# josephg/text-crdt-rust

Measured on AMD Instinct MI355X. Metric: CRDT ops remapped+merged/sec (whole node), higher is better.
Workload: dtype u32

## Files before the change

include/crdt_gpu.h:

```cpp
#ifndef CRDT_GPU_H
#define CRDT_GPU_H
#include <stddef.h>
#include <stdint.h>

#ifdef __cplusplus
extern "C" {
#endif

#define CRDT_OK 0
#define CRDT_ERR_POS_OOB -1
#define CRDT_ERR_SEQ -2
#define CRDT_ERR_UNKNOWN_AGENT -3
#define CRDT_ERR_UNKNOWN_ID -4
#define CRDT_ERR_NONTERMINATING -5
#define CRDT_ERR_CAPACITY -6
#define CRDT_ERR_EMPTY_TXN -7
#define CRDT_ERR_FRONTIER -8
#define CRDT_ERR_BAD_INPUT -9
#define CRDT_ERR_INTERNAL -10

#define CRDT_E_ARG -100
#define CRDT_E_DEVICE -101
#define CRDT_E_NOMEM -102
#define CRDT_E_WIRE -103
// ... 160 lines not shown

int crdt_doc_len(crdt_engine* e, uint64_t n, const uint32_t* doc, uint32_t* len);
int crdt_doc_status(crdt_engine* e, int32_t* status );
int crdt_digest(crdt_engine* e, uint64_t* per_doc );
int crdt_canon_counts(crdt_engine* e, uint32_t* per_doc );

int crdt_export_sizes(crdt_engine* e, uint32_t doc, uint64_t* sizes);
int crdt_export(crdt_engine* e, uint32_t doc, uint32_t* raw4, uint32_t* leaf_sizes, uint32_t* canon4,
                uint32_t* cwo4, uint32_t* del3, uint32_t* dd3, uint32_t* txn5, uint32_t* parents,
                uint32_t* frontier);

int crdt_fit(crdt_engine* e);
int crdt_fit_note(crdt_engine* e, int apply);
int crdt_reseed_random_async(crdt_engine* e, uint64_t seed, uint64_t id_base);
int crdt_digest_dev_async(crdt_engine* e, uint64_t* dev_out);
int crdt_set_share_streams(crdt_engine* e, int on);
int crdt_set_device_intern(crdt_engine* e, int on);
enum { CRDT_QUERY_LDS = 0, CRDT_QUERY_PER_THREAD = 1, CRDT_QUERY_MERGE = 2 };
int crdt_set_query_kernel(crdt_engine* e, int mode);
int crdt_set_fused_publish(crdt_engine* e, int on);
int crdt_fused_publish_stats(crdt_engine* e, uint64_t* launches, uint8_t* per_doc);
enum { CRDT_BALANCE_OFF = 0, CRDT_BALANCE_ON = 1, CRDT_BALANCE_AUTO = 2, CRDT_BALANCE_ROTATE = 3 };
int crdt_set_replay_balance(crdt_engine* e, int mode);
#define CRDT_BALANCE_BOARD_WORDS (16384u * 16u)
int crdt_debug_balance_board(crdt_engine* e, uint32_t* board, uint32_t* stamp, int* policy);
int crdt_debug_vpos(crdt_engine* e, uint32_t doc, uint32_t* vpos);
int crdt_debug_publish_plan(crdt_engine* e, uint8_t* plan, uint32_t* words);
uint64_t crdt_mem_bytes(const crdt_engine* e);
int crdt_device_bytes(uint64_t* current, uint64_t* peak, int reset_peak);
int crdt_test_fail_alloc_after(long long k);
typedef struct { uint32_t pos, agent, seq; } crdt_probe;
typedef struct { uint32_t agent, seq, pos, deleted; } crdt_probe_answer;
int crdt_apply_local_probed(crdt_engine* e, uint64_t n_docs, const uint32_t* docs, const uint64_t* txn_off,
                            const crdt_local_txn* txns, const crdt_local_op* ops, const crdt_probe* probes,
                            crdt_probe_answer* answers, int32_t* doc_status);
int crdt_debug_state(crdt_engine* e, uint32_t doc, uint32_t* out23);
int crdt_last_timings(crdt_engine* e, double* replay_ms, double* publish_ms);
void* crdt_stream(crdt_engine* e);
const char* crdt_last_error(void);
const char* crdt_build_id(void);

#ifdef __cplusplus
}
#endif
#endif
```

text-crdt-rust_amd/crdt_amd/__init__.py:

```python
from __future__ import annotations

import ctypes as C
import os
import subprocess
from typing import Iterable, Sequence

import numpy as np

PKG_DIR = os.path.dirname(os.path.abspath(__file__))
PKG_ROOT = os.path.dirname(PKG_DIR)
REPO = os.path.dirname(PKG_ROOT)
LIB_PATH = os.path.join(PKG_ROOT, "build", "libcrdt_gpu.so")
CSRC = os.path.join(PKG_ROOT, "csrc")
INCLUDE = os.path.join(REPO, "include")

OK = 0
STATUS_NAMES = {0: "OK", -1: "POS_OOB", -2: "SEQ", -3: "UNKNOWN_AGENT", -4: "UNKNOWN_ID", -5: "NONTERMINATING",
                -6: "CAPACITY", -7: "EMPTY_TXN", -8: "FRONTIER", -9: "BAD_INPUT", -10: "INTERNAL"}
ROOT_AGENT = 0xFFFF
ROOT_ORDER = 0xFFFFFFFF


class CrdtError(RuntimeError):
    pass
# ... 25 lines not shown
    if not force and os.path.exists(out) and os.path.exists(stamp):
        with open(stamp) as f:
            if f.read().strip() == hsh:
                return out
    os.makedirs(os.path.dirname(out), exist_ok=True)
    cmd = _build_cmd(out, list(defines) + [f'CRDT_SRC_HASH="{hsh}"'])
    r = subprocess.run(cmd, capture_output=not verbose, text=True)
    if r.returncode != 0:
        raise CrdtError("hipcc failed:\n" + (r.stderr or "")[-4000:])
    if not defines:
        check_codegen(out + ".tmp")
    os.replace(out + ".tmp", out)
    with open(stamp, "w") as f:
        f.write(hsh + "\n")
    return out


def build_id(path: str = None) -> str:
    L = lib() if path is None else C.CDLL(path)
    L.crdt_build_id.restype = C.c_char_p
    return L.crdt_build_id().decode()


SCRATCH_STORES_MAX = {"k_replay": 4}
CODEGEN_LIMITS = {
    "k_replay": {"vgpr_count": 64, "vgpr_spill_count": 16, "private_segment_fixed_size": 32},
    "k_replay_hr": {"vgpr_count": 128, "vgpr_spill_count": 0, "private_segment_fixed_size": 0},
    "k_publish": {"vgpr_count": 64, "vgpr_spill_count": 0, "private_segment_fixed_size": 0},
}
LLVM_BIN = "/opt/rocm/lib/llvm/bin"


def kernel_resources(lib_path: str) -> dict:
    import re
    import tempfile
    import shutil
    with tempfile.TemporaryDirectory() as td:
        cp = os.path.join(td, "lib.so")
        shutil.copyfile(lib_path, cp)
        r = subprocess.run([os.path.join(LLVM_BIN, "llvm-objdump"), "--offloading", cp], capture_output=True, text=True)
        cos = [f for f in os.listdir(td) if "amdgcn-amd-amdhsa--gfx950" in f]
        if r.returncode != 0 or not cos:
            raise CrdtError("no gfx950 code object in " + lib_path + ": " + (r.stderr or "")[-500:])
        notes = subprocess.run([os.path.join(LLVM_BIN, "llvm-readelf"), "--notes", os.path.join(td, cos[0])],
                               capture_output=True, text=True, check=True).stdout
    out, cur = {}, {}
    for line in notes.splitlines():
        m = re.match(r"\s*-?\s*\.(\w+):\s+(\S+)\s*$", line)
        if not m:
# ... 95 lines not shown
    L.crdt_apply_remote_wire.argtypes = [vp, u64, P(u32), P(C.c_char_p), P(u64), P(i32)]
    L.crdt_stage_remote_wire.argtypes = [vp, u64, P(u32), P(C.c_char_p), P(u64)]
    L.crdt_stage_remote_replicated.argtypes = [vp, C.c_char_p, u64, u32, P(C.c_char_p)]
    L.crdt_stage_random.argtypes = [vp, u64, P(u32), C.c_char_p, u32, u64]
    L.crdt_stage_local_shared.argtypes = [vp, u64, P(u32), P(u32), u32, P(u64), vp, vp]
    L.crdt_debug_state.argtypes = [vp, u32, P(u32)]
    L.crdt_fit.argtypes = [vp]
    for f, at in (("crdt_fit_note", [vp, C.c_int]), ("crdt_test_fail_alloc_after", [C.c_longlong]),
                  ("crdt_reseed_random_async", [vp, u64, u64]), ("crdt_digest_dev_async", [vp, vp])):
        if hasattr(L, f):
            getattr(L, f).argtypes = at
    L.crdt_set_share_streams.argtypes = [vp, C.c_int]
    for f in ("crdt_set_device_intern", "crdt_set_query_kernel", "crdt_set_fused_publish"):
        if hasattr(L, f):
            getattr(L, f).argtypes = [vp, C.c_int]
    if hasattr(L, "crdt_fused_publish_stats"):
        L.crdt_fused_publish_stats.argtypes = [vp, P(u64), P(C.c_uint8)]
        L.crdt_debug_vpos.argtypes = [vp, u32, P(u32)]
    if hasattr(L, "crdt_debug_publish_plan"):
        L.crdt_debug_publish_plan.argtypes = [vp, P(C.c_uint8), P(u32)]
    if hasattr(L, "crdt_set_replay_balance"):
        L.crdt_set_replay_balance.argtypes = [vp, C.c_int]
        L.crdt_debug_balance_board.argtypes = [vp, P(u32), P(u32), P(C.c_int)]
    L.crdt_apply_local_probed.argtypes = [vp, u64, P(u32), P(u64), vp, vp, vp, vp, P(i32)]
    L.crdt_mem_bytes.argtypes = [vp]
    L.crdt_mem_bytes.restype = u64
    if hasattr(L, "crdt_device_bytes"):
        L.crdt_device_bytes.argtypes = [P(u64), P(u64), C.c_int]
    L.crdt_reset_async.argtypes = [vp]
    L.crdt_run.argtypes = [vp, P(i32)]
    L.crdt_run_async.argtypes = [vp]
    L.crdt_publish_async.argtypes = [vp]
    L.crdt_sync.argtypes = [vp]
    L.crdt_pos_to_loc.argtypes = [vp, u64, P(u32), P(u32), P(C.c_uint16), P(u32)]
    L.crdt_loc_to_pos.argtypes = [vp, u64, P(u32), P(C.c_uint16), P(u32), P(u32), P(C.c_uint8)]
    L.crdt_pos_to_loc_dev_async.argtypes = [vp, u64, vp, vp, vp, vp]
    L.crdt_loc_to_pos_dev_async.argtypes = [vp, u64, vp, vp, vp, vp, vp]
    L.crdt_doc_len.argtypes = [vp, u64, P(u32), P(u32)]
    L.crdt_doc_status.argtypes = [vp, P(i32)]
    L.crdt_digest.argtypes = [vp, P(u64)]
    if hasattr(L, "crdt_canon_counts"):
        L.crdt_canon_counts.argtypes = [vp, P(u32)]
    L.crdt_export_sizes.argtypes = [vp, u32, P(u64)]
    L.crdt_export.argtypes = [vp, u32] + [P(u32)] * 9
    L.crdt_last_timings.argtypes = [vp, P(C.c_double), P(C.c_double)]
    L.crdt_stream.argtypes = [vp]
# ... 68 lines not shown

EXPORTED_SYMBOLS = [
    "crdt_engine_create", "crdt_engine_destroy", "crdt_docs_alloc", "crdt_num_docs", "crdt_agent_intern", "crdt_agent_intern_dev",
    "crdt_apply_local", "crdt_apply_remote_wire", "crdt_stage_local", "crdt_stage_remote_wire",
    "crdt_stage_remote_replicated", "crdt_reset_async", "crdt_run", "crdt_run_async", "crdt_publish_async",
    "crdt_sync", "crdt_pos_to_loc", "crdt_loc_to_pos", "crdt_pos_to_loc_dev_async", "crdt_loc_to_pos_dev_async",
    "crdt_doc_len", "crdt_doc_status", "crdt_digest", "crdt_export_sizes", "crdt_export", "crdt_last_timings",
    "crdt_stream", "crdt_last_error", "crdt_build_id", "crdt_stage_random", "crdt_debug_state",
    "crdt_stage_local_shared", "crdt_set_content", "crdt_materialize_async", "crdt_text", "crdt_text_digest",
    "crdt_last_materialize_ms", "crdt_set_content_copies", "crdt_canon_counts", "crdt_fit", "crdt_mem_bytes", "crdt_apply_local_probed", "crdt_set_share_streams", "crdt_set_device_intern", "crdt_set_query_kernel", "crdt_device_bytes",
    "crdt_fit_note", "crdt_reseed_random_async", "crdt_digest_dev_async", "crdt_test_fail_alloc_after",
    "crdt_doc_version", "crdt_diff_async", "crdt_diff_between_async", "crdt_diff_counts", "crdt_diff_read", "crdt_last_diff_ms",
    "crdt_checkout_async", "crdt_checkout_lens", "crdt_checkout_read", "crdt_checkout_digest", "crdt_pos_to_loc_at",
    "crdt_loc_to_pos_at", "crdt_pos_to_loc_at_dev_async", "crdt_loc_to_pos_at_dev_async", "crdt_last_checkout_ms",
    "crdt_blame_async", "crdt_blame_counts", "crdt_blame_read", "crdt_last_blame_ms",
    "crdt_encode_async", "crdt_encode_lens", "crdt_encode_read", "crdt_pos_to_units", "crdt_units_to_pos",
    "crdt_pos_to_units_dev_async", "crdt_units_to_pos_dev_async", "crdt_last_encode_ms",
    "crdt_lines_async", "crdt_line_counts", "crdt_lines_read", "crdt_pos_to_linecol", "crdt_linecol_to_pos",
    "crdt_pos_to_linecol_dev_async", "crdt_linecol_to_pos_dev_async", "crdt_last_lines_ms",
    "crdt_find_async", "crdt_find_counts", "crdt_find_read", "crdt_find_seek", "crdt_find_seek_dev_async", "crdt_last_find_ms",
    "crdt_edits_async", "crdt_edits_counts", "crdt_edits_read", "crdt_last_edits_ms",
    "crdt_rebase_async", "crdt_rebase_counts", "crdt_rebase_read", "crdt_rebase", "crdt_rebase_dev_async", "crdt_last_rebase_ms",
    "crdt_set_fused_publish", "crdt_fused_publish_stats", "crdt_debug_vpos", "crdt_debug_publish_plan",
    "crdt_set_replay_balance", "crdt_debug_balance_board",
    "crdt_trace_load", "crdt_trace_parse", "crdt_trace_sizes", "crdt_trace_copy", "crdt_trace_free",
]


def _p(a, t=C.c_uint32):
    return a.ctypes.data_as(C.POINTER(t))


def _check(rc: int, what: str):
    if rc != 0:
        err = lib().crdt_last_error()
        raise CrdtError(f"{what} failed rc={rc} {err.decode() if err else ''}")


class Engine:

    def __init__(self, n_docs: int, leaf_cap: int = 32, device: int = 0):
        L = lib()
        self.L = L
        self.h = C.c_void_p()
        cfg = L.Cfg(leaf_cap, device)
        _check(L.crdt_engine_create(C.byref(cfg), C.byref(self.h)), "crdt_engine_create")
        _check(L.crdt_docs_alloc(self.h, n_docs), "crdt_docs_alloc")
# ... 150 lines not shown

    QUERY_KERNELS = {"lds": 0, "per_thread": 1, "merge": 2}

    def query_kernel(self, mode: str):
        _check(self.L.crdt_set_query_kernel(self.h, self.QUERY_KERNELS[mode]), "query_kernel")

    def device_intern(self, on: bool = True):
        _check(self.L.crdt_set_device_intern(self.h, int(on)), "device_intern")

    def fused_publish(self, on: bool = True):
        _check(self.L.crdt_set_fused_publish(self.h, int(on)), "fused_publish")

    def fused_publish_stats(self):
        n = C.c_uint64()
        per = np.zeros(self.n_docs, np.uint8)
        _check(self.L.crdt_fused_publish_stats(self.h, C.byref(n), _p(per, C.c_uint8)), "fused_publish_stats")
        return n.value, per.astype(bool)

    BALANCE_MODES = {"off": 0, "on": 1, "auto": 2, "rotate": 3}

    def replay_balance(self, mode="auto"):
        _check(self.L.crdt_set_replay_balance(self.h, int(self.BALANCE_MODES.get(mode, mode))), "replay_balance")

    def balance_board(self):
        board = np.zeros((16384, 16), np.uint32)
        stamp, policy = C.c_uint32(), C.c_int()
        _check(self.L.crdt_debug_balance_board(self.h, _p(board), C.byref(stamp), C.byref(policy)), "debug_balance_board")
        return board, stamp.value, policy.value

    def debug_vpos(self, doc: int) -> np.ndarray:
        out = np.zeros(max(int(self.canon_counts()[doc]), 1), np.uint32)
        _check(self.L.crdt_debug_vpos(self.h, doc, _p(out)), "debug_vpos")
        return out[: int(self.canon_counts()[doc])]

    def publish_plan(self):
        plan = np.zeros(self.n_docs, np.uint8)
        words = np.zeros(self.n_docs, np.uint32)
        _check(self.L.crdt_debug_publish_plan(self.h, _p(plan, C.c_uint8), _p(words)), "debug_publish_plan")
        return plan, words

    def mem_bytes(self) -> int:
        return int(self.L.crdt_mem_bytes(self.h))

    @staticmethod
    def device_bytes(reset_peak: bool = False):
        cur, peak = C.c_uint64(), C.c_uint64()
# ... 610 lines not shown
```

text-crdt-rust_amd/csrc/engine.hip:

```cpp
#include <hip/hip_runtime.h>

#include <algorithm>
#include <cstdio>
#include <cstring>
#include <map>
#include <mutex>
#include <string>
#include <unordered_map>
#include <vector>

#include "crdt_gpu.h"
#include "host_plan.h"
#include "kernels.h"
#include "encode.h"
#include "lines.h"
#include "find.h"
#include "edits.h"
#include "rebase.h"

using namespace crdt;

namespace {

thread_local std::string g_last_error;
// ... 285 lines not shown
  u64* cbase = nullptr;
  u64* clen = nullptr;
  u32* text = nullptr;
  u64 text_cap = 0;
  u64 ord_total = 0;
  Span* canon = nullptr;
  u32* vpos = nullptr;
  u32* sorted = nullptr;
  u32* corder = nullptr;
  u32* pub = nullptr;
  u64 canon_alloc = 0, pub_alloc = 0;
  bool pub_sized = false;
  bool pub_fitted = false;
  std::vector<u32> pub_small, pub_big;
  u32* pub_list = nullptr;
  u32 pubx_words = 0;
  u32* stamp = nullptr;
  u64 fused_launches = 0;
  u32 state_id = 1;
  bool fused_publish = !(getenv("CRDT_NO_FUSED_PUBLISH") && getenv("CRDT_NO_FUSED_PUBLISH")[0] == '1');
  u32* bal_board = nullptr;
  int replay_balance = getenv("CRDT_REPLAY_BALANCE") && getenv("CRDT_REPLAY_BALANCE")[0] >= '0' && getenv("CRDT_REPLAY_BALANCE")[0] <= '3'
                           ? getenv("CRDT_REPLAY_BALANCE")[0] - '0' : CRDT_BALANCE_AUTO;
  u32 n_cus = 0;
  u32 bal_last_stamp = 0, bal_last_mode = BAL_OFF;
  u32 balance_mode(const RootClass& c, const LaunchShape& sh) const {
    if (replay_balance == CRDT_BALANCE_OFF) return BAL_OFF;
    if (replay_balance == CRDT_BALANCE_ROTATE) return BAL_ROTATE;
    if (replay_balance == CRDT_BALANCE_ON) return BAL_BOARD;
    const u64 by_regs = 4ull * (c.shape == SHAPE_GEN ? CRDT_REPLAY_WAVES_GEN : CRDT_REPLAY_WAVES);
    const u64 by_lds = (163840ull / std::max<size_t>(sh.lds, 1)) * sh.wpb;
    return c.n <= std::min(by_regs, by_lds) * n_cus ? BAL_ROTATE : BAL_OFF;
  }
  void state_changed() {
    if (++state_id == STAMP_BIG) {
      state_id = 1;
      pub_sized = pub_fitted = false;
    }
  }
  u32* tlen = nullptr;
  u64* tdigest = nullptr;
  bool materialized = false;
  void* qbuf = nullptr;
  u64 qbuf_bytes = 0;
  ResultJob<DiffRes, 2> diff;
  std::vector<u32> diff_docs_h, diff_since_h, diff_to_h;
// ... 640 lines not shown
    return 0;
  }

  int launch_replay() {
    if (!n_docs) return 0;
    Pools pv = pools_view(pools);
    state_changed();
    bal_last_stamp = state_id % 255u + 1u;
    bal_last_mode = BAL_OFF;
    const bool fuse = fused_publish && pub_sized && pub_fitted;
    for (const RootClass& c : classes) {
      LaunchShape sh = launch_shape(c.rcap, c.hr);
      u32 blocks = (u32)((c.n + sh.wpb - 1) / sh.wpb);
      const u32* list = c.off == INVALID ? nullptr : doc_list + c.off;
      if (c.hr) {
        if (L == 32) hipLaunchKernelGGL(k_replay_hr<32>, dim3(blocks), dim3(64 * sh.wpb), sh.lds, stream, pv, (u32)c.n, sh.wpb, sh.rcap, list);
        else hipLaunchKernelGGL(k_replay_hr<4>, dim3(blocks), dim3(64 * sh.wpb), sh.lds, stream, pv, (u32)c.n, sh.wpb, sh.rcap, list);
      } else {
        const u32 bal = balance_mode(c, sh);
        bal_last_mode = std::max(bal_last_mode, bal);
        ReplayArgs ra{pv, (u32)c.n, sh.wpb, sh.rcap, list, pub_view(), pubx_words, fuse ? state_id : 0u,
                      bal_board, bal_last_stamp, bal};
        if (L == 32) {
          if (c.shape == SHAPE_REMOTE) hipLaunchKernelGGL((k_replay<32, SHAPE_REMOTE>), dim3(blocks), dim3(64 * sh.wpb), sh.lds, stream, ra);
          else if (c.shape == SHAPE_GEN) hipLaunchKernelGGL((k_replay<32, SHAPE_GEN>), dim3(blocks), dim3(64 * sh.wpb), sh.lds, stream, ra);
          else if (c.shape == SHAPE_LOCAL) hipLaunchKernelGGL((k_replay<32, SHAPE_LOCAL>), dim3(blocks), dim3(64 * sh.wpb), sh.lds, stream, ra);
          else hipLaunchKernelGGL((k_replay<32, SHAPE_ALL>), dim3(blocks), dim3(64 * sh.wpb), sh.lds, stream, ra);
        } else {
          if (c.shape == SHAPE_REMOTE) hipLaunchKernelGGL((k_replay<4, SHAPE_REMOTE>), dim3(blocks), dim3(64 * sh.wpb), sh.lds, stream, ra);
          else if (c.shape == SHAPE_GEN) hipLaunchKernelGGL((k_replay<4, SHAPE_GEN>), dim3(blocks), dim3(64 * sh.wpb), sh.lds, stream, ra);
          else if (c.shape == SHAPE_LOCAL) hipLaunchKernelGGL((k_replay<4, SHAPE_LOCAL>), dim3(blocks), dim3(64 * sh.wpb), sh.lds, stream, ra);
          else hipLaunchKernelGGL((k_replay<4, SHAPE_ALL>), dim3(blocks), dim3(64 * sh.wpb), sh.lds, stream, ra);
        }
      }
      HIPCHK(hipGetLastError());
    }
    for (const RootClass& c : classes) if (fuse && !c.hr) { fused_launches++; break; }
    if (!pub_fitted) pub_sized = false;
    published = false;
    materialized = false;
    return 0;
  }

  int pull_states() {
    HIPCHK(hipMemcpyAsync(st_h.data(), st, n_docs * sizeof(DocState), hipMemcpyDeviceToHost, stream));
    HIPCHK(hipStreamSynchronize(stream));
    return 0;
  }

  int run(int32_t* status_out) {
    int r = set_device();
    if (r) return r;
// ... 891 lines not shown
  *out = nullptr;
  int n = 0;
  if (hipGetDeviceCount(&n) != hipSuccess || n <= cfg->device || cfg->device < 0) return CRDT_E_DEVICE;
  hipDeviceProp_t prop;
  if (hipGetDeviceProperties(&prop, cfg->device) != hipSuccess) return CRDT_E_DEVICE;
  if (std::strncmp(prop.gcnArchName, "gfx950", 6) != 0) return CRDT_E_DEVICE;
  crdt_engine* e = new crdt_engine();
  e->L = cfg->leaf_cap;
  e->device = cfg->device;
  bool ok = hipSetDevice(e->device) == hipSuccess && hipStreamCreateWithFlags(&e->stream, hipStreamNonBlocking) == hipSuccess;
  for (auto& x : e->ev) ok = ok && hipEventCreate(&x) == hipSuccess;
  e->each_job([&](auto& j) { ok = ok && j.create(e->device, e->stream) == 0; });
  e->n_cus = (u32)prop.multiProcessorCount;
  ok = ok && hipMalloc((void**)&e->bal_board, (size_t)BAL_ROWS * BAL_SLOTS * 4) == hipSuccess &&
       hipMemsetAsync(e->bal_board, 0, (size_t)BAL_ROWS * BAL_SLOTS * 4, e->stream) == hipSuccess;
  if (!ok) {
    crdt_engine_destroy(e);
    return CRDT_E_DEVICE;
  }
  (void)hipFuncSetAttribute((const void*)k_replay<32, SHAPE_ALL>, hipFuncAttributeMaxDynamicSharedMemorySize, 163840);
  (void)hipFuncSetAttribute((const void*)k_replay<4, SHAPE_ALL>, hipFuncAttributeMaxDynamicSharedMemorySize, 163840);
  (void)hipFuncSetAttribute((const void*)k_replay<32, SHAPE_REMOTE>, hipFuncAttributeMaxDynamicSharedMemorySize, 163840);
  (void)hipFuncSetAttribute((const void*)k_replay<4, SHAPE_REMOTE>, hipFuncAttributeMaxDynamicSharedMemorySize, 163840);
  (void)hipFuncSetAttribute((const void*)k_replay<32, SHAPE_GEN>, hipFuncAttributeMaxDynamicSharedMemorySize, 163840);
  (void)hipFuncSetAttribute((const void*)k_replay<32, SHAPE_LOCAL>, hipFuncAttributeMaxDynamicSharedMemorySize, 163840);
  (void)hipFuncSetAttribute((const void*)k_replay<4, SHAPE_GEN>, hipFuncAttributeMaxDynamicSharedMemorySize, 163840);
  (void)hipFuncSetAttribute((const void*)k_replay<4, SHAPE_LOCAL>, hipFuncAttributeMaxDynamicSharedMemorySize, 163840);
  (void)hipFuncSetAttribute((const void*)k_replay_hr<32>, hipFuncAttributeMaxDynamicSharedMemorySize, 163840);
  (void)hipFuncSetAttribute((const void*)k_replay_hr<4>, hipFuncAttributeMaxDynamicSharedMemorySize, 163840);
  (void)hipFuncSetAttribute((const void*)k_pos_to_loc_blk<32>, hipFuncAttributeMaxDynamicSharedMemorySize, QBLK_LDS);
  (void)hipFuncSetAttribute((const void*)k_pos_to_loc_blk<4>, hipFuncAttributeMaxDynamicSharedMemorySize, QBLK_LDS);
  (void)hipFuncSetAttribute((const void*)k_loc_to_pos_blk<32>, hipFuncAttributeMaxDynamicSharedMemorySize, QBLK_W * 8u);
  (void)hipFuncSetAttribute((const void*)k_loc_to_pos_blk<4>, hipFuncAttributeMaxDynamicSharedMemorySize, QBLK_W * 8u);
  (void)hipFuncSetAttribute((const void*)k_pub_index, hipFuncAttributeMaxDynamicSharedMemorySize,
                            (int)pubx_lds_bytes(PUBX_MAX_WORDS));
  (void)hipFuncSetAttribute((const void*)k_diff_mark, hipFuncAttributeMaxDynamicSharedMemorySize, (int)(DIFF_MARK_WORDS * 4u));
  *out = e;
  return 0;
}

void crdt_engine_destroy(crdt_engine* e) {
  if (!e) return;
  (void)hipSetDevice(e->device);
  if (e->stream) (void)hipStreamSynchronize(e->stream);
  e->release();
  if (e->bal_board) (void)hipFree(e->bal_board);
// ... 403 lines not shown
  if (!e) return CRDT_E_ARG;
  e->share_streams = on != 0;
  return 0;
}

int crdt_set_query_kernel(crdt_engine* e, int mode) {
  if (!e || mode < CRDT_QUERY_LDS || mode > CRDT_QUERY_MERGE) return CRDT_E_ARG;
  e->query_kernel = mode;
  return 0;
}

int crdt_set_fused_publish(crdt_engine* e, int on) {
  if (!e) return CRDT_E_ARG;
  e->fused_publish = on != 0;
  return 0;
}

int crdt_set_replay_balance(crdt_engine* e, int mode) {
  if (!e || mode < CRDT_BALANCE_OFF || mode > CRDT_BALANCE_ROTATE) return CRDT_E_ARG;
  e->replay_balance = mode;
  return 0;
}

int crdt_debug_balance_board(crdt_engine* e, uint32_t* board, uint32_t* stamp, int* policy) {
  if (poisoned(e)) return CRDT_E_NOMEM;
  if (!valid(e)) return CRDT_E_ARG;
  if (stamp) *stamp = e->bal_last_stamp;
  if (policy) *policy = (int)e->bal_last_mode;
  if (board) {
    HIPCHK(hipMemcpyAsync(board, e->bal_board, (size_t)BAL_ROWS * BAL_SLOTS * 4, hipMemcpyDeviceToHost, e->stream));
    HIPCHK(hipStreamSynchronize(e->stream));
  }
  return 0;
}

int crdt_fused_publish_stats(crdt_engine* e, uint64_t* launches, uint8_t* per_doc) {
  if (poisoned(e)) return CRDT_E_NOMEM;
  if (!valid(e)) return CRDT_E_ARG;
  if (launches) *launches = e->fused_launches;
  if (per_doc && e->n_docs) {
    std::vector<u32> st(e->n_docs);
    HIPCHK(hipMemcpyAsync(st.data(), e->stamp, e->n_docs * 4, hipMemcpyDeviceToHost, e->stream));
    HIPCHK(hipStreamSynchronize(e->stream));
    for (u64 d = 0; d < e->n_docs; d++) per_doc[d] = st[d] == e->state_id;
  }
  return 0;
// ... 1167 lines not shown
```

text-crdt-rust_amd/csrc/kernels.h:

```cpp
#pragma once
#include "replay_core.h"
#include "wave_gpu.h"

namespace crdt {

struct PubOut {
  Span* canon;
  u32* vpos;
  u32* sorted;
  u32* corder;
  u32* pub;
  u32* canon_n;
  u32* len;
  u64* digest;
  u32* stamp;
};
constexpr u32 STAMP_BIG = 0xFFFFFFFFu;

#ifdef PUB_PLAIN_LOADS
__device__ __forceinline__ u32 ld_l2(const u32* p) { return *p; }
#else
__device__ __forceinline__ u32 ld_l2(const u32* p) { return __hip_atomic_load(p, __ATOMIC_RELAXED, __HIP_MEMORY_SCOPE_AGENT); }
#endif
__device__ __forceinline__ u32 span_of_order(const PubOut& O, const DocSeg& seg, u32 cn, u32 order) {
// ... 34 lines not shown
  u32 d;
  if (!wave_doc(wpb, nullptr, n, d)) return;
  Replayer<WaveGPU<L>, L> r(P, d, wave_with_root<L>(rcap));
  r.init_empty();
  AgentRec* ag = r.agents();
  for (u32 a = lane_id(); a < r.g(S_N_AGENTS); a += 64) ag[a].run_cnt = 0;
  r.finish();
}

struct ReplayArgs {
  Pools P;
  u32 n, wpb, rcap;
  const u32* list;
  PubOut O;
  u32 xw, pub_id;
  u32* bal_board;
  u32 bal_stamp;
  u32 bal_mode;
};
template <int L>
__device__ __forceinline__ void publish_tail(const DocState* stp);
__device__ __forceinline__ void balance_done();

template <int L, bool HR, u32 SH = SHAPE_ALL, bool FUSE = false>
__device__ __forceinline__ void replay_doc(Pools P, u32 n, u32 wpb, u32 rcap, const u32* list) {
  u32 d;
  if (!wave_doc(wpb, list, n, d)) return;
#ifdef CRDT_PROF
  const u32 life_t0 = (u32)__builtin_amdgcn_s_memrealtime();
#endif
  Replayer<WaveGPU<L, HR>, L> r(P, d, wave_with_root<L, HR>(rcap));
  WaveGPU<L, HR>& w = r.w;
  if (r.status() == ST_NEED_CAPACITY) r.p(S_STATUS, (u32)ST_OK);
  if (r.status() != ST_OK || r.g(S_REC_POS) >= r.rec_n()) {
    w.st((u32*)&P.st[d].status, (u32)r.status());
    if constexpr (!HR) balance_done();
    return;
  }
  r.begin();
  r.template run<SH>();
  r.finish();
#ifdef CRDT_PROF
  __builtin_amdgcn_fence(__ATOMIC_RELEASE, "workgroup");
  const u32 life_t1 = (u32)__builtin_amdgcn_s_memrealtime();
#endif
  if constexpr (!HR) balance_done();
  if constexpr (FUSE) publish_tail<L>(r.stp());
#ifdef CRDT_PROF
  if (r.prof_mode == 4u) {
    __builtin_amdgcn_fence(__ATOMIC_RELEASE, "workgroup");
    const u32 tail = (u32)__builtin_amdgcn_s_memrealtime() - life_t1;
    w.st(&P.st[d].prof0, life_t0);
    w.st(&P.st[d].prof1, life_t1);
    w.st(&P.st[d].prof2, (u32)__builtin_amdgcn_s_getreg(4 | (31 << 11)));
    w.st(&P.st[d].prof3, ((u32)__builtin_amdgcn_s_getreg(20 | (31 << 11)) & 15u) | (tail << 4));
  }
#endif
}
#ifndef CRDT_REPLAY_WAVES
#define CRDT_REPLAY_WAVES 8
#endif
#ifndef CRDT_REPLAY_WAVES_GEN
#define CRDT_REPLAY_WAVES_GEN CRDT_REPLAY_WAVES
#endif
template <int L, u32 SH>
__global__ __launch_bounds__(256) __attribute__((amdgpu_waves_per_eu(SH == SHAPE_GEN ? CRDT_REPLAY_WAVES_GEN : CRDT_REPLAY_WAVES))) void k_replay(ReplayArgs A) {
  replay_doc<L, false, SH, true>(A.P, A.n, A.wpb, A.rcap, A.list);
}
template <int L>
__global__ __launch_bounds__(256) __attribute__((amdgpu_waves_per_eu(4))) void k_replay_hr(Pools P, u32 n, u32 wpb, u32 rcap, const u32* list) {
  replay_doc<L, true>(P, n, wpb, rcap, list);
}

__global__ void k_reseed_gen(Pools P, u32 n, u64 seed, u64 id_base) {
  u32 d = blockIdx.x * blockDim.x + threadIdx.x;
  if (d >= n) return;
  DocSeg sg = P.seg[d];
  if (sg.rec_n != 1u) return;
  Rec* r = const_cast<Rec*>(P.recs + sg.rec_base);
  if (rec_kind(*r) != REC_GEN) return;
  r->w3 = (u32)mix64(seed ^ (id_base + d));
}

__global__ void k_reset_recpos(DocState* st, u32 n, u32 n_agents_dummy) {
  u32 d = blockIdx.x * blockDim.x + threadIdx.x;
  if (d < n) st[d].rec_pos = 0;
}

__global__ void k_set_n_agents(DocState* st, const u32* na, u32 n) {
  u32 d = blockIdx.x * blockDim.x + threadIdx.x;
// ... 2283 lines not shown
```

text-crdt-rust_amd/csrc/replay_core.h:

```cpp
#pragma once
#include "crdt_types.h"

namespace crdt {

struct Cursor {
  u32 leaf, idx, off;
};
constexpr u32 END_LEAF = 0xFFFFFFFEu;

enum : u32 {
  P_LV = 0, P_DL = 2, P_DV = 4, P_SOL = 6, P_LOF = 8, P_CWO = 10, P_ARUN = 12, P_DELS = 14,
  P_DD = 16, P_TXNS = 18, P_PAR = 20, P_FR = 22, P_AGENTS = 24, P_GROUPS = 26, P_RECS = 28, P_STP = 30,
  P_DDB = 32,
  P_PROBE = P_DDB + 2,
  K_LEAF = P_PROBE + 2, K_MAP, K_CWO, K_TXN, K_DEL, K_DD, K_PAR, K_RECN,
  K_FR,
  P_OAG,
  K_AGMAP = P_OAG + 2,
  P_LAG,
  S_BASE = 64,
  S_STATUS = 64, S_REC_POS, S_N_LEAVES, S_N_BLOCKS, S_NG, S_NEXT_ORDER, S_LEN, S_N_CWO, S_N_DEL,
  S_N_DD, S_N_TXN, S_N_PAR, S_N_FR, S_N_AGENTS, S_N_ITEMS, S_CAP_NEED, S_N_ENTRIES, S_GEN_DONE, S_N_DDB,
  S_PROF0, S_PROF1, S_PROF2, S_PROF3,
  F_FAST,
  F_PRE, PRE_ITEM, PRE_C = PRE_ITEM + 4,
  F_GEN = PRE_C + 3,
  T_RB_BASE,
  F_BASE,
  FR_S0 = 104,
  C_LEAF = 128, C_N, C_VIS, C_NOW, C_BLK, C_I, C_VSTART, C_DIRTY, C_VS_OK ,
  C_SUCC, C_SUCC_ORD,
  T_CWO_KEY, T_CWO_AGENT, T_CWO_SEQ, T_CWO_LEN,
  T_DEL_KEY, T_DEL_ORDER, T_DEL_LEN,
  T_TX_ORDER, T_TX_LEN, T_TX_SHADOW,
  T_FR0,
  T_AG_ID, T_AG_BASE, T_AG_CNT, T_AG_CAP,
  T_AGL_KEY, T_AGL_ORDER, T_AGL_LEN,
  T_OA_ID, T_OA_BASE, T_OA_CNT,
  T_AGP_KEY, T_AGP_ORDER, T_AGP_LEN,
  T_OA_KEY, T_OA_ORDER, T_OA_LEN,
  N_SLOTS
};
static_assert(P_LAG + 1 < 64, "read-only slots live in the first context register");
static_assert(S_PROF3 - S_BASE + 1 == sizeof(DocState) / 4, "DocState slot mirror");
static_assert(F_BASE < FR_S0, "DocState and the flags live in the second context register, below the frontier heads");
constexpr u32 FR_LANES = 128u - FR_S0;
static_assert(N_SLOTS <= 192, "three context registers");

template <class W, int L>
struct Replayer {
  W w;
  u32 cpt = 0;
  CRDT_HD u32 per_txn(u32 remote) const { return cpt ? 1u : (remote ? 3u : 2u); }
  CRDT_HD Rec op_at(u32 b, u32 remote) const {
    Rec r = w.rec_get(cpt ? b : b + 1u);
    if (!cpt) return r;
    Rec h, o, pr;
    if (remote) expand_rc(r, h, o, pr);
    else expand_lc(r, h, o);
    return o;
  }
#ifdef CRDT_PROF
  u32 prof_cat = 0;
  u32 prof_mode = 0;
  u32 prof_gen = 0;
  u32 prof_cur = 0, prof_sw = 0;
  u64 prof_t2 = 0;
  u32 prof_split = 0;
  u32 pt_scan = 0, pt_del = 0, pt_ins = 0;
#endif
#ifdef CRDT_EMU_STATS
  u32 st_prev_leaf = INVALID;
// ... 75 lines not shown
    p(K_AGMAP, (sg.flags & DOC_TRACK_AGENT) ? 1u : 0u);
    w.x_load_state(P.st + d, S_BASE);
    p(C_LEAF, INVALID);
    p(C_N, 0);
    p(C_VIS, 0);
    p(C_NOW, 0);
    p(C_BLK, 0);
    p(C_I, 0);
    p(C_VSTART, VS_BAD);
    p(C_DIRTY, 0);
    p(C_SUCC, INVALID);
    p(C_SUCC_ORD, 0);
    p(T_CWO_KEY, 0); p(T_CWO_AGENT, 0); p(T_CWO_SEQ, 0); p(T_CWO_LEN, 0);
    p(T_DEL_KEY, INVALID); p(T_DEL_ORDER, 0); p(T_DEL_LEN, 0);
    p(T_TX_ORDER, 0); p(T_TX_LEN, 0); p(T_TX_SHADOW, 0);
    p(T_FR0, ROOT_ORDER);
    p(T_AG_ID, INVALID); p(T_AG_BASE, 0); p(T_AG_CNT, 0); p(T_AG_CAP, 0);
    p(T_AGL_KEY, 0); p(T_AGL_ORDER, 0); p(T_AGL_LEN, 0); p(T_AGP_LEN, 0);
    p(T_OA_ID, INVALID); p(T_OA_BASE, 0); p(T_OA_CNT, 0);
    p(T_RB_BASE, 0x80000000u);
    p(F_FAST, 0);
    p(F_PRE, 0);
    p(F_GEN, 0);
  }

  CRDT_HD Span* leafp(u32 leaf) const { return w.template at<L>(lv(), leaf); }
  CRDT_HD u32* dleaf(u32 blk) const { return w.template at<GROUP>(dl(), blk); }
  CRDT_HD u32* dvis(u32 blk) const { return w.template at<GROUP>(dv(), blk); }

  CRDT_HD void init_empty() {
    p(S_STATUS, (u32)ST_OK);
    p(S_REC_POS, 0);
    p(S_N_LEAVES, 1);
    p(S_N_BLOCKS, 1);
    p(S_NG, 1);
    p(S_NEXT_ORDER, 0);
    p(S_LEN, 0);
    p(S_N_CWO, 0); p(S_N_DEL, 0); p(S_N_DD, 0); p(S_N_TXN, 0); p(S_N_PAR, 0);
    p(S_N_FR, 1);
    p(S_N_ITEMS, 0);
    p(S_CAP_NEED, 0);
    p(S_N_ENTRIES, 0);
    p(S_GEN_DONE, 0);
    p(S_N_DDB, 0);
    w.zero_leaf(leafp(0), L);
    lag_stale(0u);
// ... 52 lines not shown
    if (n <= FR_LANES + 1u) w.fr_lanes_store(fr(), n);
  }
  CRDT_HD void flush_agent() {
    u32 a = g(T_AG_ID), cnt = g(T_AG_CNT);
    if (a != INVALID && cnt) {
      u32 ln = g(T_AGL_LEN);
      w.st(&w.at(arun(), g(T_AG_BASE) + cnt - 1)->len, ln);
      w.st_agent_tail(w.at(agents(), a), g(T_AGL_KEY), g(T_AGL_ORDER), ln);
    }
  }
  CRDT_HD void finish() {
    commit();
    flush_tails();
    w.root_store(groups(), g(S_NG));
    w.x_store_state(stp(), S_BASE);
  }

  template <class X> static CRDT_HD auto tick_of(X& x, u32 remaining, int) -> decltype(x.balance_tick(remaining)) {
    x.balance_tick(remaining);
  }
  template <class X> static CRDT_HD void tick_of(X&, u32, long) {}
  CRDT_HD void balance_tick(u32 remaining) { tick_of(w, remaining, 0); }

  CRDT_HD void rec_window(u32 base) {
    u32 d = base - g(T_RB_BASE);
    u32 nn = rec_n() - base;
    balance_tick(nn);
    u32 ahead = nn > 64u ? nn - 64u : 0u;
    if (d <= 64u) w.rec_slide(d, recs() + base + 64u, ahead < 64u ? ahead : 64u);
    else w.rec_load2(recs() + base, nn < 64u ? nn : 64u, ahead < 64u ? ahead : 64u);
    p(T_RB_BASE, base);
  }
  CRDT_HD Rec rec(u32 pos) {
    u32 base = g(T_RB_BASE);
    u32 d = pos - base;
    if (d > 61u) rec_window(d <= 64u ? pos : (d < 125u ? base + 64u : pos));
    return w.rec_get(pos - g(T_RB_BASE));
  }
  CRDT_HD Rec rec_at(u32 pos) const {
    u32 d = pos - g(T_RB_BASE);
    return d < 64u ? w.rec_get(d) : w.ld_rec(w.at(recs(), pos));
  }

  CRDT_HD void slot_of(u32 leaf, u32& blk, u32& i) const {
    if (leaf == g(C_LEAF)) { blk = g(C_BLK); i = g(C_I); return; }
    u32 v = w.ld(w.template at<2>(sol(), leaf));
    blk = v >> 6;
    i = v & 63u;
  }
  CRDT_HD u32 pos_key(u32 leaf) const {
    u32 blk, i;
    slot_of(leaf, blk, i);
    return (w.root_find_blk(g(S_NG), blk) << 6) | i;
  }
// ... 1115 lines not shown
    if (g(T_FR0) != first - 1u) return 0;
    if (g(S_N_TXN) == 0u) return 0;
    return g(T_TX_ORDER) + g(T_TX_LEN) == first;
  }
  CRDT_HD void fast_txn_commit(u32 first, u32 len) {
    if (!g(F_FAST)) {
      p(F_BASE, first);
      p(F_FAST, 1u);
    }
    p(S_NEXT_ORDER, first + len);
    inc(T_AGL_LEN, len);
  }
  CRDT_HD u32 next_item_after(u32 idx, u32& order) {
    if (idx + 1u < g(C_N)) { order = w.cget_order(idx + 1u); return 1u; }
    u32 fo;
    u32 has = cached_succ(fo) != INVALID;
    order = fo;
    return has;
  }
  CRDT_HD u32 typing_run(u32 b0, u32 nv, u32 remote, u32 agent, u32 ow1, const Rec& o, u32& total) {
    u32 nt = 1u;
    total = remote ? (o.w0 & 0x0FFFFFFFu) : o.w3;
    if (!nv) return nt;
    nt = w.typing_scan(b0, nv, remote, cpt, agent, ow1, o.w3, total);
    u32 per = per_txn(remote), rn = rec_n();
    u32 pos0 = g(T_RB_BASE) + b0;
    u32 end = g(T_RB_BASE) + nv;
    while (true) {
      if (pos0 + (nt + 1u) * per <= end) break;
      if (end >= rn) break;
      u32 last = pos0 + (nt - 1u) * per;
      u32 n = rn - last < 64u ? rn - last : 64u;
      u32 t2, l0;
      u32 n2 = w.typing_scan_at(w.at(recs(), last), n, remote, cpt, agent, ow1, o.w3, t2, l0);
      end = last + n;
      if (n2 <= 1u) break;
      total += t2 - l0;
      nt += n2 - 1u;
    }
    return nt;
  }
  CRDT_HD u32 fast_typing(u32 b0, u32 nv, u32 remote, u32 idx, u32 orr, u32 agent, const Rec& o, u32 first) {
    Span e = w.cget(idx);
    if (e.len <= 0) return 0;
    if (e.order + (u32)e.len != first) return 0;
    if (e.orr != orr) return 0;
    u32 total;
// ... 929 lines not shown
```

text-crdt-rust_amd/csrc/wave_gpu.h:

```cpp
#pragma once
#include "crdt_types.h"

namespace crdt {

__device__ __forceinline__ u32 lane_id() { return __lane_id(); }
__device__ __forceinline__ u32 lane_here() {
  u32 l;
  asm volatile("v_mbcnt_lo_u32_b32 %0, -1, 0\n\tv_mbcnt_hi_u32_b32 %0, -1, %0" : "=v"(l));
  return l;
}
__device__ __forceinline__ u32 uni(u32 x) { return __builtin_amdgcn_readfirstlane(x); }
__device__ __forceinline__ u32 rdlane(u32 x, u32 l) { return __builtin_amdgcn_readlane(x, l); }
__device__ int crdt_writelane_i32(int v, int l, int old) __asm("llvm.amdgcn.writelane.i32");
__device__ __forceinline__ u32 wrlane(u32 old, u32 v, u32 l) { return (u32)crdt_writelane_i32((int)v, (int)l, (int)old); }
__device__ __forceinline__ u64 ballot(bool p) { return __builtin_amdgcn_ballot_w64(p); }
__device__ __forceinline__ u32 shfl(u32 v, u32 src) { return __builtin_amdgcn_ds_bpermute((int)(src << 2), (int)v); }

__device__ __forceinline__ u32 wave_umax(u32 v) {
  v = max(v, (u32)__builtin_amdgcn_update_dpp(0u, v, 0x111, 0xf, 0xf, false));
  v = max(v, (u32)__builtin_amdgcn_update_dpp(0u, v, 0x112, 0xf, 0xf, false));
  v = max(v, (u32)__builtin_amdgcn_update_dpp(0u, v, 0x114, 0xf, 0xf, false));
  v = max(v, (u32)__builtin_amdgcn_update_dpp(0u, v, 0x118, 0xf, 0xf, false));
  v = max(v, (u32)__builtin_amdgcn_update_dpp(0u, v, 0x142, 0xa, 0xf, false));
  v = max(v, (u32)__builtin_amdgcn_update_dpp(0u, v, 0x143, 0xc, 0xf, false));
// ... 659 lines not shown
    u32 l = lane();
    u32 d = (rx ^ ((REC_LC << 28) | agent)) | ry | rz | (rw ^ len);
    u64 stop = ballot(d != 0u || l >= nv) & (~1ull << b0);
    u32 f = stop ? (u32)__builtin_ctzll(stop) : 64u;
    return f - b0;
  }
  __device__ __forceinline__ u32 typing_scan(u32 b0, u32 nv, u32 remote, u32 compact, u32 agent, u32 ow1, u32 ow3,
                                             u32& total) const {
    return typing_scan_r(rx, ry, rz, rw, b0, nv, remote, compact, agent, ow1, ow3, total);
  }
  __device__ __forceinline__ u32 typing_scan_at(const Rec* p, u32 nv, u32 remote, u32 compact, u32 agent, u32 ow1,
                                                u32 ow3, u32& total, u32& len0) const {
    uint4 v = rec_lane_load(p, nv);
    len0 = (compact & remote) ? (rdlane(v.x, 0) >> 16) & 0x7FFu : rdlane(v.w, 0);
    return typing_scan_r(v.x, v.y, v.z, v.w, 0u, nv, remote, compact, agent, ow1, ow3, total);
  }
  __device__ __forceinline__ u32 delete_scan(u32 b0, u32 nv, u32 remote, u32 compact, u32 agent, u32 delta) const {
    return delete_scan_r(rx, ry, rz, rw, b0, nv, remote, compact, agent, delta);
  }
  __device__ __forceinline__ u32 delete_scan_at(const Rec* p, u32 nv, u32 remote, u32 compact, u32 agent, u32 delta) const {
    uint4 v = rec_lane_load(p, nv);
    return delete_scan_r(v.x, v.y, v.z, v.w, 0u, nv, remote, compact, agent, delta);
  }
  __device__ __forceinline__ u32 frontier_advance(u32* f, u32 nfr, u32 f0, const u32* pp, u32 np, u32 p0, u32 first,
                                                  u32 last, u32 cap, u32& nf0) const {
    u32 l = lane();
    bool in = l < nfr;
    u32 fv = f[in ? l : 0u];
    fv = l == 0u ? f0 : fv;
    if (ballot(in && fv == first)) return 0u;
    u32 pv = np > 1u ? pp[l < np ? l : 0u] : 0u;
    pv = l == 0u ? p0 : pv;
    bool hit = false;
    for (u32 j = 0; j < np; j++) hit |= fv == rdlane(pv, j);
    u64 keep = ballot(in && !hit);
    u32 m = (u32)__popcll(keep);
    if (m + 1u > cap) return INVALID;
    nf0 = m ? rdlane(fv, (u32)__builtin_ctzll(keep)) : last;
    u32 at = (u32)__popcll(keep & ((1ull << l) - 1ull));
    if (((keep >> l) & 1ull) && at >= 1u) f[at] = fv;
    if (m) f[m] = last;
    return m + 1u;
  }
  static constexpr u32 FR_L0 = FR_S0 - 64u;
  __device__ __forceinline__ void fr_lanes_load(const u32* f, u32 n) {
    u32 l = lane();
// ... 462 lines not shown
```

Baseline: 33.48 billion.

## Precompute typing-run mask per record window in remote replay kernel

Adds a remote-only replay kernel variant that, each time the record window is loaded or slid, compares every lane's record with its neighbour via DPP and ballots a bitmask of records that continue a typing run. The mask is stored in context-register slots. For compact remote ops the typing scan then finds the run length with a count-trailing-zeros on that mask instead of running the full per-op typing scan. This trades some extra work per window refill for cheaper scans per op, and adds a new kernel instance with its own register budget. It is on by default and can be turned off with an environment variable.

Result: faster. 34.27 billion (median of 6 runs) (+2.4%).

```diff
diff --git a/include/crdt_gpu.h b/include/crdt_gpu.h
--- a/include/crdt_gpu.h
+++ b/include/crdt_gpu.h
@@ -206,6 +206,7 @@
 int crdt_fused_publish_stats(crdt_engine* e, uint64_t* launches, uint8_t* per_doc);
 enum { CRDT_BALANCE_OFF = 0, CRDT_BALANCE_ON = 1, CRDT_BALANCE_AUTO = 2, CRDT_BALANCE_ROTATE = 3 };
 int crdt_set_replay_balance(crdt_engine* e, int mode);
+int crdt_set_window_decode(crdt_engine* e, int on);
 #define CRDT_BALANCE_BOARD_WORDS (16384u * 16u)
 int crdt_debug_balance_board(crdt_engine* e, uint32_t* board, uint32_t* stamp, int* policy);
 int crdt_debug_vpos(crdt_engine* e, uint32_t doc, uint32_t* vpos);
diff --git a/text-crdt-rust_amd/crdt_amd/__init__.py b/text-crdt-rust_amd/crdt_amd/__init__.py
--- a/text-crdt-rust_amd/crdt_amd/__init__.py
+++ b/text-crdt-rust_amd/crdt_amd/__init__.py
@@ -71,9 +71,10 @@
     return L.crdt_build_id().decode()
 
 
-SCRATCH_STORES_MAX = {"k_replay": 4}
+SCRATCH_STORES_MAX = {"k_replay": 4, "k_replay_dec": 0}
 CODEGEN_LIMITS = {
     "k_replay": {"vgpr_count": 64, "vgpr_spill_count": 16, "private_segment_fixed_size": 32},
+    "k_replay_dec": {"vgpr_count": 64, "vgpr_spill_count": 0, "private_segment_fixed_size": 0},
     "k_replay_hr": {"vgpr_count": 128, "vgpr_spill_count": 0, "private_segment_fixed_size": 0},
     "k_publish": {"vgpr_count": 64, "vgpr_spill_count": 0, "private_segment_fixed_size": 0},
 }
@@ -215,6 +216,8 @@
     if hasattr(L, "crdt_set_replay_balance"):
         L.crdt_set_replay_balance.argtypes = [vp, C.c_int]
         L.crdt_debug_balance_board.argtypes = [vp, P(u32), P(u32), P(C.c_int)]
+    if hasattr(L, "crdt_set_window_decode"):
+        L.crdt_set_window_decode.argtypes = [vp, C.c_int]
     L.crdt_apply_local_probed.argtypes = [vp, u64, P(u32), P(u64), vp, vp, vp, vp, P(i32)]
     L.crdt_mem_bytes.argtypes = [vp]
     L.crdt_mem_bytes.restype = u64
@@ -329,7 +332,7 @@
     "crdt_edits_async", "crdt_edits_counts", "crdt_edits_read", "crdt_last_edits_ms",
     "crdt_rebase_async", "crdt_rebase_counts", "crdt_rebase_read", "crdt_rebase", "crdt_rebase_dev_async", "crdt_last_rebase_ms",
     "crdt_set_fused_publish", "crdt_fused_publish_stats", "crdt_debug_vpos", "crdt_debug_publish_plan",
-    "crdt_set_replay_balance", "crdt_debug_balance_board",
+    "crdt_set_replay_balance", "crdt_debug_balance_board", "crdt_set_window_decode",
     "crdt_trace_load", "crdt_trace_parse", "crdt_trace_sizes", "crdt_trace_copy", "crdt_trace_free",
 ]
 
@@ -526,6 +529,9 @@
     def replay_balance(self, mode="auto"):
         _check(self.L.crdt_set_replay_balance(self.h, int(self.BALANCE_MODES.get(mode, mode))), "replay_balance")
 
+    def window_decode(self, on=True):
+        _check(self.L.crdt_set_window_decode(self.h, int(on)), "window_decode")
+
     def balance_board(self):
         board = np.zeros((16384, 16), np.uint32)
         stamp, policy = C.c_uint32(), C.c_int()
diff --git a/text-crdt-rust_amd/csrc/engine.hip b/text-crdt-rust_amd/csrc/engine.hip
--- a/text-crdt-rust_amd/csrc/engine.hip
+++ b/text-crdt-rust_amd/csrc/engine.hip
@@ -331,6 +331,7 @@
   u32* bal_board = nullptr;
   int replay_balance = getenv("CRDT_REPLAY_BALANCE") && getenv("CRDT_REPLAY_BALANCE")[0] >= '0' && getenv("CRDT_REPLAY_BALANCE")[0] <= '3'
                            ? getenv("CRDT_REPLAY_BALANCE")[0] - '0' : CRDT_BALANCE_AUTO;
+  bool window_decode = !(getenv("CRDT_WINDOW_DECODE") && getenv("CRDT_WINDOW_DECODE")[0] == '0');
   u32 n_cus = 0;
   u32 bal_last_stamp = 0, bal_last_mode = BAL_OFF;
   u32 balance_mode(const RootClass& c, const LaunchShape& sh) const {
@@ -1017,12 +1018,14 @@
         ReplayArgs ra{pv, (u32)c.n, sh.wpb, sh.rcap, list, pub_view(), pubx_words, fuse ? state_id : 0u,
                       bal_board, bal_last_stamp, bal};
         if (L == 32) {
-          if (c.shape == SHAPE_REMOTE) hipLaunchKernelGGL((k_replay<32, SHAPE_REMOTE>), dim3(blocks), dim3(64 * sh.wpb), sh.lds, stream, ra);
+          if (c.shape == SHAPE_REMOTE && window_decode) hipLaunchKernelGGL((k_replay_dec<32>), dim3(blocks), dim3(64 * sh.wpb), sh.lds, stream, ra);
+          else if (c.shape == SHAPE_REMOTE) hipLaunchKernelGGL((k_replay<32, SHAPE_REMOTE>), dim3(blocks), dim3(64 * sh.wpb), sh.lds, stream, ra);
           else if (c.shape == SHAPE_GEN) hipLaunchKernelGGL((k_replay<32, SHAPE_GEN>), dim3(blocks), dim3(64 * sh.wpb), sh.lds, stream, ra);
           else if (c.shape == SHAPE_LOCAL) hipLaunchKernelGGL((k_replay<32, SHAPE_LOCAL>), dim3(blocks), dim3(64 * sh.wpb), sh.lds, stream, ra);
           else hipLaunchKernelGGL((k_replay<32, SHAPE_ALL>), dim3(blocks), dim3(64 * sh.wpb), sh.lds, stream, ra);
         } else {
-          if (c.shape == SHAPE_REMOTE) hipLaunchKernelGGL((k_replay<4, SHAPE_REMOTE>), dim3(blocks), dim3(64 * sh.wpb), sh.lds, stream, ra);
+          if (c.shape == SHAPE_REMOTE && window_decode) hipLaunchKernelGGL((k_replay_dec<4>), dim3(blocks), dim3(64 * sh.wpb), sh.lds, stream, ra);
+          else if (c.shape == SHAPE_REMOTE) hipLaunchKernelGGL((k_replay<4, SHAPE_REMOTE>), dim3(blocks), dim3(64 * sh.wpb), sh.lds, stream, ra);
           else if (c.shape == SHAPE_GEN) hipLaunchKernelGGL((k_replay<4, SHAPE_GEN>), dim3(blocks), dim3(64 * sh.wpb), sh.lds, stream, ra);
           else if (c.shape == SHAPE_LOCAL) hipLaunchKernelGGL((k_replay<4, SHAPE_LOCAL>), dim3(blocks), dim3(64 * sh.wpb), sh.lds, stream, ra);
           else hipLaunchKernelGGL((k_replay<4, SHAPE_ALL>), dim3(blocks), dim3(64 * sh.wpb), sh.lds, stream, ra);
@@ -1960,6 +1963,8 @@
   (void)hipFuncSetAttribute((const void*)k_replay<4, SHAPE_ALL>, hipFuncAttributeMaxDynamicSharedMemorySize, 163840);
   (void)hipFuncSetAttribute((const void*)k_replay<32, SHAPE_REMOTE>, hipFuncAttributeMaxDynamicSharedMemorySize, 163840);
   (void)hipFuncSetAttribute((const void*)k_replay<4, SHAPE_REMOTE>, hipFuncAttributeMaxDynamicSharedMemorySize, 163840);
+  (void)hipFuncSetAttribute((const void*)k_replay_dec<32>, hipFuncAttributeMaxDynamicSharedMemorySize, 163840);
+  (void)hipFuncSetAttribute((const void*)k_replay_dec<4>, hipFuncAttributeMaxDynamicSharedMemorySize, 163840);
   (void)hipFuncSetAttribute((const void*)k_replay<32, SHAPE_GEN>, hipFuncAttributeMaxDynamicSharedMemorySize, 163840);
   (void)hipFuncSetAttribute((const void*)k_replay<32, SHAPE_LOCAL>, hipFuncAttributeMaxDynamicSharedMemorySize, 163840);
   (void)hipFuncSetAttribute((const void*)k_replay<4, SHAPE_GEN>, hipFuncAttributeMaxDynamicSharedMemorySize, 163840);
@@ -2409,6 +2414,12 @@
   return 0;
 }
 
+int crdt_set_window_decode(crdt_engine* e, int on) {
+  if (!e) return CRDT_E_ARG;
+  e->window_decode = on != 0;
+  return 0;
+}
+
 int crdt_debug_balance_board(crdt_engine* e, uint32_t* board, uint32_t* stamp, int* policy) {
   if (poisoned(e)) return CRDT_E_NOMEM;
   if (!valid(e)) return CRDT_E_ARG;
diff --git a/text-crdt-rust_amd/csrc/kernels.h b/text-crdt-rust_amd/csrc/kernels.h
--- a/text-crdt-rust_amd/csrc/kernels.h
+++ b/text-crdt-rust_amd/csrc/kernels.h
@@ -80,14 +80,15 @@
 __device__ __forceinline__ void publish_tail(const DocState* stp);
 __device__ __forceinline__ void balance_done();
 
-template <int L, bool HR, u32 SH = SHAPE_ALL, bool FUSE = false>
+template <int L, bool HR, u32 SH = SHAPE_ALL, bool FUSE = false, bool DEC = false>
 __device__ __forceinline__ void replay_doc(Pools P, u32 n, u32 wpb, u32 rcap, const u32* list) {
   u32 d;
   if (!wave_doc(wpb, list, n, d)) return;
 #ifdef CRDT_PROF
   const u32 life_t0 = (u32)__builtin_amdgcn_s_memrealtime();
 #endif
-  Replayer<WaveGPU<L, HR>, L> r(P, d, wave_with_root<L, HR>(rcap));
+  static_assert(!DEC || (!HR && SH == SHAPE_REMOTE), "the window decode is built into the remote-only instance");
+  Replayer<WaveGPU<L, HR>, L, DEC> r(P, d, wave_with_root<L, HR>(rcap));
   WaveGPU<L, HR>& w = r.w;
   if (r.status() == ST_NEED_CAPACITY) r.p(S_STATUS, (u32)ST_OK);
   if (r.status() != ST_OK || r.g(S_REC_POS) >= r.rec_n()) {
@@ -124,6 +125,10 @@
 template <int L, u32 SH>
 __global__ __launch_bounds__(256) __attribute__((amdgpu_waves_per_eu(SH == SHAPE_GEN ? CRDT_REPLAY_WAVES_GEN : CRDT_REPLAY_WAVES))) void k_replay(ReplayArgs A) {
   replay_doc<L, false, SH, true>(A.P, A.n, A.wpb, A.rcap, A.list);
+}
+template <int L>
+__global__ __launch_bounds__(256) __attribute__((amdgpu_waves_per_eu(CRDT_REPLAY_WAVES))) void k_replay_dec(ReplayArgs A) {
+  replay_doc<L, false, SHAPE_REMOTE, true, true>(A.P, A.n, A.wpb, A.rcap, A.list);
 }
 template <int L>
 __global__ __launch_bounds__(256) __attribute__((amdgpu_waves_per_eu(4))) void k_replay_hr(Pools P, u32 n, u32 wpb, u32 rcap, const u32* list) {
diff --git a/text-crdt-rust_amd/csrc/replay_core.h b/text-crdt-rust_amd/csrc/replay_core.h
--- a/text-crdt-rust_amd/csrc/replay_core.h
+++ b/text-crdt-rust_amd/csrc/replay_core.h
@@ -39,15 +39,17 @@
   T_OA_ID, T_OA_BASE, T_OA_CNT,
   T_AGP_KEY, T_AGP_ORDER, T_AGP_LEN,
   T_OA_KEY, T_OA_ORDER, T_OA_LEN,
-  N_SLOTS
+  W_TYP,
+  N_SLOTS = W_TYP + 2
 };
 static_assert(P_LAG + 1 < 64, "read-only slots live in the first context register");
 static_assert(S_PROF3 - S_BASE + 1 == sizeof(DocState) / 4, "DocState slot mirror");
 static_assert(F_BASE < FR_S0, "DocState and the flags live in the second context register, below the frontier heads");
 constexpr u32 FR_LANES = 128u - FR_S0;
 static_assert(N_SLOTS <= 192, "three context registers");
-
-template <class W, int L>
+static_assert(W_TYP >= 128, "the window mask lives in the third context register");
+
+template <class W, int L, bool DEC = false>
 struct Replayer {
   W w;
   u32 cpt = 0;
@@ -169,6 +171,7 @@
     p(F_FAST, 0);
     p(F_PRE, 0);
     p(F_GEN, 0);
+    p(W_TYP, 0); p(W_TYP + 1, 0);
   }
 
   CRDT_HD Span* leafp(u32 leaf) const { return w.template at<L>(lv(), leaf); }
@@ -267,6 +270,10 @@
   template <class X> static CRDT_HD void tick_of(X&, u32, long) {}
   CRDT_HD void balance_tick(u32 remaining) { tick_of(w, remaining, 0); }
 
+  template <class X> static constexpr auto has_decode_of(int) -> decltype(&X::decode_window, &X::win_mask, true) { return true; }
+  template <class X> static constexpr bool has_decode_of(long) { return false; }
+  static constexpr bool has_decode = DEC && has_decode_of<W>(0);
+
   CRDT_HD void rec_window(u32 base) {
     u32 d = base - g(T_RB_BASE);
     u32 nn = rec_n() - base;
@@ -275,6 +282,7 @@
     if (d <= 64u) w.rec_slide(d, recs() + base + 64u, ahead < 64u ? ahead : 64u);
     else w.rec_load2(recs() + base, nn < 64u ? nn : 64u, ahead < 64u ? ahead : 64u);
     p(T_RB_BASE, base);
+    if constexpr (has_decode) w.decode_window(nn < 64u ? nn : 64u, W_TYP);
   }
   CRDT_HD Rec rec(u32 pos) {
     u32 base = g(T_RB_BASE);
@@ -1436,7 +1444,12 @@
     u32 nt = 1u;
     total = remote ? (o.w0 & 0x0FFFFFFFu) : o.w3;
     if (!nv) return nt;
-    nt = w.typing_scan(b0, nv, remote, cpt, agent, ow1, o.w3, total);
+    bool decoded = false;
+    if constexpr (has_decode) {
+      decoded = (cpt & remote) != 0u;
+      if (decoded) nt = w.typing_scan_m(b0, W_TYP, total);
+    }
+    if (!decoded) nt = w.typing_scan(b0, nv, remote, cpt, agent, ow1, o.w3, total);
     u32 per = per_txn(remote), rn = rec_n();
     u32 pos0 = g(T_RB_BASE) + b0;
     u32 end = g(T_RB_BASE) + nv;
diff --git a/text-crdt-rust_amd/csrc/wave_gpu.h b/text-crdt-rust_amd/csrc/wave_gpu.h
--- a/text-crdt-rust_amd/csrc/wave_gpu.h
+++ b/text-crdt-rust_amd/csrc/wave_gpu.h
@@ -705,6 +705,32 @@
     uint4 v = rec_lane_load(p, nv);
     return delete_scan_r(v.x, v.y, v.z, v.w, 0u, nv, remote, compact, agent, delta);
   }
+  __device__ __forceinline__ static u32 wave_shr1(u32 v) {
+    u32 r = (u32)__builtin_amdgcn_update_dpp(0, (int)v, 0x138, 0xf, 0xf, false);
+    asm("" : "+v"(r));
+    return r;
+  }
+  __device__ __forceinline__ void decode_window(u32 nv, u32 s_typ) {
+    u32 l = lane();
+    u32 p0 = wave_shr1(rx), p1 = wave_shr1(ry), p3 = wave_shr1(rw);
+    u32 dt = ((rx & RC_HDR_MASK) ^ ((REC_RC << 28) | (p0 & 0xFFFFu))) | (ry ^ (p1 + ((p0 >> 16) & 0x7FFu))) |
+             (rz ^ (ry - 1u)) | (rw ^ p3);
+    bool in = l - 1u < nv - 1u;
+    u64 mt = ballot(in & (dt == 0u) & ((rx & (0x7FFu << 16)) != 0u));
+    xs(s_typ, (u32)mt); xs(s_typ + 1u, (u32)(mt >> 32));
+  }
+  __device__ __forceinline__ u64 win_mask(u32 s) const { return ((u64)rdlane(x2, s - 127u) << 32) | rdlane(x2, s - 128u); }
+  __device__ __forceinline__ static u32 mask_run(u64 m, u32 b0) {
+    u64 stop = ~m & (~1ull << b0);
+    return (stop ? (u32)__builtin_ctzll(stop) : 64u) - b0;
+  }
+  __device__ __forceinline__ u32 typing_scan_m(u32 b0, u32 s_typ, u32& total) const {
+    u32 n = mask_run(win_mask(s_typ), b0);
+    u32 e = b0 + n - 1u;
+    total = rdlane(ry, e) + ((rdlane(rx, e) >> 16) & 0x7FFu) - rdlane(ry, b0);
+    return n;
+  }
+
   __device__ __forceinline__ u32 frontier_advance(u32* f, u32 nfr, u32 f0, const u32* pp, u32 np, u32 p0, u32 first,
                                                   u32 last, u32 cap, u32& nf0) const {
     u32 l = lane();
```
